# JihyongOh/DeMFI

Measured on AMD Instinct MI355X. Metric: interpolated frames/sec @720p x8 MFI (N_tst=3), higher is better.
Workload: dtype f16

## Files before the change

demfi_amd/csrc/conv_wstream.hip:

```cpp
#include "conv_common.h"

namespace {

#ifndef DEMFI_WS3_DEPTH
#define DEMFI_WS3_DEPTH 9
#endif
#ifndef DEMFI_WS_NW
#define DEMFI_WS_NW 4
#endif
template <int KS, int NW, int NCH = 2, int TH_ = 16> struct WsCfg {
    static constexpr int TH = TH_;
    static constexpr int RPW = TH / (NW / NCH);
    static constexpr int BL = KS + RPW - 1;
    static constexpr int LH = TH + KS - 1;
    static constexpr int LL = KS == 7 ? ((TW + KS - 1 + 7) & ~7) : TW + KS - 1;
    static constexpr int NI = (LH * LL + 15) / 16;
    static constexpr int UNIT_BYTES = NI * 1024;
    static constexpr int LDS_BYTES = 2 * UNIT_BYTES;
    static constexpr int NG = 2 * KS;
    static constexpr int NSTEP = NG * KS;
    static constexpr int DEPTH = NW == 8 ? KS : (KS == 7 ? 2 * KS : DEMFI_WS3_DEPTH);
    static constexpr int NIW = (NI + NW - 1) / NW;
    static constexpr int DMA_EVERY = KS == 7 ? 6 : 1;
    static constexpr int DMA_PER = KS == 7 ? 1 : 3;
    static constexpr bool PIECE_STRIDES = KS != 7;
    static_assert(LDS_BYTES <= 160 * 1024, "two units must fit LDS");
    static_assert((NIW + DMA_PER - 1) / DMA_PER * DMA_EVERY + DEPTH <= NSTEP, "the unit's DMA must be older than the last A fragment consumed in the unit");
    static_assert(NSTEP % DEPTH == 0, "static ring indices");
};

template <int KS, int NW, int NCH = 2, int TH_ = 16>
__global__ __launch_bounds__(64 * NW, 1) void conv_wstream_c64_kernel(const demfi_conv* __restrict__ d)
{
    using C = WsCfg<KS, NW, NCH, TH_>;
    constexpr int WS_TH = C::TH;
    constexpr int RPW = C::RPW;
    extern __shared__ __attribute__((aligned(16))) char smem[];
    const int tid = threadIdx.x;
    const int lane = tid & 63;
    const int wave = __builtin_amdgcn_readfirstlane(tid >> 6);
    const int hi = lane >> 5, lx = lane & 31;
    const int cs = NCH == 2 ? (wave & 1) : 0, rh = NCH == 2 ? (wave >> 1) : wave;
    const int H = d->H, W = d->W;
    const int tiles_x = (W + TW - 1) / TW, tiles_y = (H + WS_TH - 1) / WS_TH, tiles_img = tiles_x * tiles_y;
    const int total = tiles_img * d->batch;
    int t_first, t_end, t_step;
    {
        const int G = gridDim.x;
        if ((G & 7) == 0 && total >= G) {
            const int xcd = blockIdx.x & 7, idx = blockIdx.x >> 3;
            const int q = (total + 7) >> 3, lo = xcd * q;
            t_first = lo + idx;
            t_end = min(lo + q, total);
            t_step = G >> 3;
        } else {
            t_first = blockIdx.x;
            t_end = total;
            t_step = G;
        }
    }
    if (t_first >= t_end) return;
    const int upt = d->n_chunks;
    const int n_units = ((t_end - t_first + t_step - 1) / t_step) * upt;

    const demfi_piece& p0 = d->pieces[d->chunks[0].first_piece];
    const int64_t sxb = p0.v.sx * 2, syb = p0.v.sy * 2, sbb = p0.v.sb * 2;
    const char* const zeros = (const char*)d->zero_page;
    const uint4* const wbase = (const uint4*)d->wpack;

    int doff[C::NIW], dlc[C::NIW];
#pragma unroll
    for (int j = 0; j < C::NIW; ++j) {
        const int rec = min((wave + NW * j) * 16 + (lane >> 2), C::LH * C::LL - 1);
        const int l = rec / C::LL, c = rec - l * C::LL;
        doff[j] = C::PIECE_STRIDES ? (((lane & 3) ^ ((c >> 2) & 3)) << 4) : (int)(l * syb + c * sxb) + (((lane & 3) ^ ((c >> 2) & 3)) << 4);
        dlc[j] = l | (c << 8);
    }
    int boff[C::NG];
#pragma unroll
    for (int g = 0; g < C::NG; ++g) {
        const int col = lx + (g >> 1);
        boff[g] = (rh * RPW * C::LL + col) * 64 + ((((g & 1) * 2 + hi) ^ ((col >> 2) & 3)) << 4);
    }

    struct Unit { const char* src; const char* w; int iy0, ix0; bool interior; int sx, sy; };
    const unsigned lane16 = lane * 16;
    auto unit_info = [&](int u) {
        Unit r;
        const int k = u / upt, cu = u - k * upt;
        const int it = t_first + k * t_step;
        const int bimg = it / tiles_img, rem = it - bimg * tiles_img;
        const int ty = rem / tiles_x, tx = rem - ty * tiles_x;
        r.iy0 = ty * WS_TH - KS / 2;
        r.ix0 = tx * TW - KS / 2;
        const demfi_piece& pc = d->pieces[d->chunks[cu].first_piece];
        r.sx = C::PIECE_STRIDES ? (int)(pc.v.sx * 2) : (int)sxb;
        r.sy = C::PIECE_STRIDES ? (int)(pc.v.sy * 2) : (int)syb;
        r.src = (const char*)pc.v.ptr + bimg * (C::PIECE_STRIDES ? pc.v.sb * 2 : sbb) + (int64_t)r.iy0 * r.sy + (int64_t)r.ix0 * r.sx;
        r.w = (const char*)(wbase + d->chunks[cu].w_off + cs * 64);
        r.interior = r.iy0 >= 0 && r.iy0 + C::LH <= H && r.ix0 >= 0 && r.ix0 + C::LL <= W;
        return r;
    };
    auto dma_one = [&](auto J, const Unit& un, char* buf) {
        constexpr int j = decltype(J)::value;
        const int i = wave + NW * j;
        if (i >= C::NI) return;
        const char* g = un.src + doff[j];
        if constexpr (C::PIECE_STRIDES) g += (dlc[j] & 255) * un.sy + (dlc[j] >> 8) * un.sx;
        if (!un.interior) {
            const int iy = un.iy0 + (dlc[j] & 255), ix = un.ix0 + (dlc[j] >> 8);
            if (!(iy >= 0 && iy < H && ix >= 0 && ix < W)) g = zeros;
        }
        const unsigned la = (unsigned)(uintptr_t)(__attribute__((address_space(3))) char*)(buf + i * 1024);
#if defined(__HIP_DEVICE_COMPILE__)
        unsigned m0_save;
        asm volatile("s_mov_b32 %0, m0\n\ts_mov_b32 m0, %2\n\ts_nop 0\n\tglobal_load_lds_dwordx4 %1, off\n\ts_mov_b32 m0, %0"
                     : "=&s"(m0_save) : "v"(g), "s"(la) : "memory");
#endif
    };
    auto a_load = [&](const Unit& un, int t) {
        const int g = t / KS, ky = t - g * KS, kx = g >> 1, ksl = g & 1;
        return __builtin_bit_cast(uint4, *gcp<u4_t>(un.w + (unsigned)((((ky * KS + kx) * 2 + ksl) * NCH) * 1024 + lane16)));
    };

    const demfi_seg& sg = d->segs[d->sub_seg[0]];
    half_t* const dstp = (half_t*)sg.dst.ptr;
    const int act = sg.act;
    const int ch0 = d->oct_ch[0];
    f4_t bq[4];
#pragma unroll
    for (int qd = 0; qd < 4; ++qd) bq[qd] = *gcp<f4_t>(d->bias + cs * 32 + qd * 8 + hi * 4);

    f16x_t acc[RPW];
#pragma unroll
    for (int p = 0; p < RPW; ++p) {
#pragma unroll
        for (int i = 0; i < 16; ++i) acc[p][i] = 0.0f;
    }
    uint4 A[C::DEPTH];
    Unit cur = unit_info(0);
    static_for<0, C::NIW>([&](auto J) { dma_one(J, cur, smem); });
    static_for<0, C::DEPTH>([&](auto T) { A[decltype(T)::value] = a_load(cur, decltype(T)::value); });
    asm volatile("s_waitcnt vmcnt(%0)" ::"n"(C::DEPTH) : "memory");
    asm volatile("s_barrier" ::: "memory");

    for (int u = 0; u < n_units; ++u) {
        const bool has_next = u + 1 < n_units;
        TRACE_STAMP(wave, u / upt, u % upt);
        const Unit nxt = unit_info(has_next ? u + 1 : 0);
        const char* const tb = smem + (u & 1) * C::UNIT_BYTES;
        char* const nb = smem + ((u + 1) & 1) * C::UNIT_BYTES;
        uint4 B[2][C::BL];
#pragma unroll
        for (int r = 0; r < RPW; ++r) B[0][r] = *(const uint4*)(tb + boff[0] + r * (C::LL * 64));
        __builtin_amdgcn_sched_barrier(0);
        static_for<0, C::NSTEP>([&](auto T_) {
            constexpr int t = decltype(T_)::value;
            constexpr int g = t / KS, ky = t % KS, gb = g & 1;
            const uint4 a = A[t % C::DEPTH];
            if constexpr (ky + RPW < C::BL) B[gb][ky + RPW] = *(const uint4*)(tb + boff[g] + (ky + RPW) * (C::LL * 64));
            if constexpr (g + 1 < C::NG) {
                if constexpr (ky < RPW) B[gb ^ 1][ky] = *(const uint4*)(tb + boff[g + 1] + ky * (C::LL * 64));
                if constexpr (ky == KS - 1) {
#pragma unroll
                    for (int r = KS; r < RPW; ++r) B[gb ^ 1][r] = *(const uint4*)(tb + boff[g + 1] + r * (C::LL * 64));
                }
            }
            if constexpr (t + C::DEPTH < C::NSTEP) A[t % C::DEPTH] = a_load(cur, t + C::DEPTH);
            else                                   A[t % C::DEPTH] = a_load(nxt, t + C::DEPTH - C::NSTEP);
            if constexpr (KS == 7) {
                if constexpr (t % C::DMA_EVERY == 2 && t / C::DMA_EVERY < C::NIW) {
                    if (has_next) dma_one(std::integral_constant<int, t / C::DMA_EVERY>{}, nxt, nb);
                }
            } else {
                if (has_next) {
                    static_for<0, C::DMA_PER>([&](auto Q) {
                        constexpr int j = t * C::DMA_PER + decltype(Q)::value;
                        if constexpr (j < C::NIW) dma_one(std::integral_constant<int, j>{}, nxt, nb);
                    });
                }
            }
#pragma unroll
            for (int p = 0; p < RPW; ++p) Mma<half_t>::run(acc[p], a, B[gb][ky + p]);
            __builtin_amdgcn_sched_barrier(0);
        });
        asm volatile("s_waitcnt vmcnt(%0)" ::"n"(C::DEPTH) : "memory");
        const int k = u / upt;
        if (u - k * upt == upt - 1) {
            const int it = t_first + k * t_step;
            const int bimg = it / tiles_img, rem = it - bimg * tiles_img;
            const int ty = rem / tiles_x, tx = rem - ty * tiles_x;
            const int ox = tx * TW + lx;
#pragma unroll
            for (int p = 0; p < RPW; ++p) {
                const int oy = ty * WS_TH + rh * RPW + p;
#pragma unroll
                for (int m2 = 0; m2 < 2; ++m2) {
                    float v[8];
#pragma unroll
                    for (int j = 0; j < 4; ++j) {
                        v[j] = acc[p][(2 * m2) * 4 + j] + bq[2 * m2][j];
                        v[4 + j] = acc[p][(2 * m2 + 1) * 4 + j] + bq[2 * m2 + 1][j];
                    }
                    apply_act_n<8>(v, act);
                    if (oy < H && ox < W)
                        store8<half_t>(dstp + bimg * sg.dst.sb + oy * sg.dst.sy + ox * sg.dst.sx + ch0 + cs * 32 + m2 * 16 + hi * 8, v);
                }
#pragma unroll
                for (int i = 0; i < 16; ++i) acc[p][i] = 0.0f;
            }
        }
        asm volatile("s_barrier" ::: "memory");
        cur = nxt;
    }
}

static bool wstream_eligible(const demfi_conv* h, int ks = 7, int nch = 2)
{
    if (h->dtype != DEMFI_F16 || h->stride != 1 || h->kh != ks || h->kw != ks || h->pad_y != ks / 2 || h->pad_x != ks / 2) return false;
    if (h->inH != h->H || h->inW != h->W || !h->zero_page || h->rec_bytes != 64) return false;
    if (h->n_chunks < (ks == 7 ? 1 : 2) || h->cout_pad != 32 * nch || h->nco != nch) return false;
    const demfi_piece& p0 = h->pieces[h->chunks[0].first_piece];
    for (int c = 0; c < h->n_chunks; ++c) {
        const demfi_chunk& ch = h->chunks[c];
        if (ch.n_pieces != 1 || ch.nks != 2) return false;
        const demfi_piece& p = h->pieces[ch.first_piece];
        if (!p.fat || p.nch != 32 || p.up_shift || !p.v.ptr || p.v.sc != 1 || p.v.is_f32) return false;
        if (ks == 7 && (p.v.sx != p0.v.sx || p.v.sy != p0.v.sy || p.v.sb != p0.v.sb)) return false;
        if (p.v.sy * 2 * 40 >= (int64_t)1 << 31 || p.v.sx * 2 * 48 >= (int64_t)1 << 31) return false;
    }
    const int sgi = h->sub_seg[0];
    if (sgi < 0 || (nch == 2 && (h->sub_seg[1] != sgi || h->oct_ch[4] != h->oct_ch[0] + 32))) return false;
    for (int o = 0; o < 4 * nch; ++o)
        if (h->oct_seg[o] != sgi || h->oct_n[o] != 8 || h->oct_ch[o] != h->oct_ch[0] + 8 * o) return false;
    const demfi_seg& sg = h->segs[sgi];
    if (sg.mode != DEMFI_MODE_STORE || sg.scale != 1 || sg.dy || sg.dx || sg.res.ptr || !sg.dst.ptr || sg.dst.is_f32 || sg.dst.sc != 1) return false;
    return true;
}

static int launch_wstream3(const demfi_conv* h, const demfi_conv* dev, hipStream_t st)
{
    DEMFI_LDS_ATTR((conv_wstream_c64_kernel<3, 4, 1, 32>));
    const int total = ((h->W + TW - 1) / TW) * ((h->H + 31) / 32) * h->batch;
    const int grid = total >= 256 ? 256 : total;
    constexpr size_t lds = WsCfg<3, 4, 1, 32>::LDS_BYTES;
    hipLaunchKernelGGL((conv_wstream_c64_kernel<3, 4, 1, 32>), dim3(grid), dim3(256), lds, st, dev);
    DEMFI_HIP_CHECK(hipGetLastError());
    return DEMFI_OK;
}

static int launch_wstream(const demfi_conv* h, const demfi_conv* dev, hipStream_t st)
{
    DEMFI_LDS_ATTR((conv_wstream_c64_kernel<7, DEMFI_WS_NW>));
    const int total = ((h->W + TW - 1) / TW) * ((h->H + 15) / 16) * h->batch;
    const int grid = total >= 256 ? 256 : total;
    constexpr size_t lds = WsCfg<7, DEMFI_WS_NW>::LDS_BYTES;
    hipLaunchKernelGGL((conv_wstream_c64_kernel<7, DEMFI_WS_NW>), dim3(grid), dim3(64 * DEMFI_WS_NW), lds, st, dev);
    DEMFI_HIP_CHECK(hipGetLastError());
    return DEMFI_OK;
}


}

DEMFI_TU_TRACE(demfi_wstream_trace_collect)

bool demfi_wstream_eligible(const demfi_conv* h, int ks, int nch) { return wstream_eligible(h, ks, nch); }
int demfi_wstream_launch(const demfi_conv* h, const demfi_conv* dev, hipStream_t st) { return launch_wstream(h, dev, st); }
int demfi_wstream3_launch(const demfi_conv* h, const demfi_conv* dev, hipStream_t st) { return launch_wstream3(h, dev, st); }
```

Before: 105.0.

## Switch wstream conv to 16x16x32 MFMA with per-kx A-fragment prefetch queue

Replaces the 32x32 MFMA tiling of the 7x7/3x3 c64 streaming conv with 16x16x32 f16 MFMAs, splitting each wave's output into two 16-column halves and two 16-channel blocks. Weight (A) fragments are now loaded per kx column as a full set of 2*KS fragments, held in a lookahead queue of LA kx steps instead of the old per-step ring of DEPTH. Lane-to-channel mapping, B offsets, bias loads and the epilogue store are remapped to match, with 4-wide half stores. This aims for better MFMA/LDS scheduling and latency hiding, at the cost of more MFMA instructions, more A registers, and narrower output stores.

```diff
diff --git a/demfi_amd/csrc/conv_wstream.hip b/demfi_amd/csrc/conv_wstream.hip
--- a/demfi_amd/csrc/conv_wstream.hip
+++ b/demfi_amd/csrc/conv_wstream.hip
@@ -2,9 +2,6 @@
 
 namespace {
 
-#ifndef DEMFI_WS3_DEPTH
-#define DEMFI_WS3_DEPTH 9
-#endif
 #ifndef DEMFI_WS_NW
 #define DEMFI_WS_NW 4
 #endif
@@ -19,15 +16,21 @@
     static constexpr int LDS_BYTES = 2 * UNIT_BYTES;
     static constexpr int NG = 2 * KS;
     static constexpr int NSTEP = NG * KS;
-    static constexpr int DEPTH = NW == 8 ? KS : (KS == 7 ? 2 * KS : DEMFI_WS3_DEPTH);
+    static constexpr int NFR = 2 * KS;
+    static constexpr int LA = NW == 8 ? 1 : (KS == 7 ? 1 : 2);
     static constexpr int NIW = (NI + NW - 1) / NW;
     static constexpr int DMA_EVERY = KS == 7 ? 6 : 1;
     static constexpr int DMA_PER = KS == 7 ? 1 : 3;
     static constexpr bool PIECE_STRIDES = KS != 7;
     static_assert(LDS_BYTES <= 160 * 1024, "two units must fit LDS");
-    static_assert((NIW + DMA_PER - 1) / DMA_PER * DMA_EVERY + DEPTH <= NSTEP, "the unit's DMA must be older than the last A fragment consumed in the unit");
-    static_assert(NSTEP % DEPTH == 0, "static ring indices");
+    static_assert(((NIW + DMA_PER - 1) / DMA_PER - 1) * DMA_EVERY + (KS == 7 ? 2 : 0) + LA * NFR <= NSTEP,
+                  "the unit's DMA must be older than the next unit's A fragments loaded in this unit");
 };
+
+__device__ __forceinline__ void mma16(f4_t& acc, const uint4& a, const uint4& b)
+{
+    acc = __builtin_amdgcn_mfma_f32_16x16x32_f16(__builtin_bit_cast(h8_t, a), __builtin_bit_cast(h8_t, b), acc, 0, 0, 0);
+}
 
 template <int KS, int NW, int NCH = 2, int TH_ = 16>
 __global__ __launch_bounds__(64 * NW, 1) void conv_wstream_c64_kernel(const demfi_conv* __restrict__ d)
@@ -35,11 +38,12 @@
     using C = WsCfg<KS, NW, NCH, TH_>;
     constexpr int WS_TH = C::TH;
     constexpr int RPW = C::RPW;
+    constexpr int LA = C::LA, NFR = C::NFR;
     extern __shared__ __attribute__((aligned(16))) char smem[];
     const int tid = threadIdx.x;
     const int lane = tid & 63;
     const int wave = __builtin_amdgcn_readfirstlane(tid >> 6);
-    const int hi = lane >> 5, lx = lane & 31;
+    const int q4 = lane >> 4, l16 = lane & 15;
     const int cs = NCH == 2 ? (wave & 1) : 0, rh = NCH == 2 ? (wave >> 1) : wave;
     const int H = d->H, W = d->W;
     const int tiles_x = (W + TW - 1) / TW, tiles_y = (H + WS_TH - 1) / WS_TH, tiles_img = tiles_x * tiles_y;
@@ -79,12 +83,12 @@
     int boff[C::NG];
 #pragma unroll
     for (int g = 0; g < C::NG; ++g) {
-        const int col = lx + (g >> 1);
-        boff[g] = (rh * RPW * C::LL + col) * 64 + ((((g & 1) * 2 + hi) ^ ((col >> 2) & 3)) << 4);
+        const int col = (g & 1) * 16 + l16 + (g >> 1);
+        boff[g] = (rh * RPW * C::LL + col) * 64 + ((q4 ^ ((col >> 2) & 3)) << 4);
     }
 
     struct Unit { const char* src; const char* w; int iy0, ix0; bool interior; int sx, sy; };
-    const unsigned lane16 = lane * 16;
+    const unsigned aoff = (unsigned)((q4 >> 1) * NCH * 1024 + (l16 + 32 * (q4 & 1)) * 16);
     auto unit_info = [&](int u) {
         Unit r;
         const int k = u / upt, cu = u - k * upt;
@@ -118,30 +122,34 @@
                      : "=&s"(m0_save) : "v"(g), "s"(la) : "memory");
 #endif
     };
-    auto a_load = [&](const Unit& un, int t) {
-        const int g = t / KS, ky = t - g * KS, kx = g >> 1, ksl = g & 1;
-        return __builtin_bit_cast(uint4, *gcp<u4_t>(un.w + (unsigned)((((ky * KS + kx) * 2 + ksl) * NCH) * 1024 + lane16)));
+    auto a_load = [&](const Unit& un, int kx, int f) {
+        const int ky = f >> 1, cb = f & 1;
+        return __builtin_bit_cast(uint4, *gcp<u4_t>(un.w + (unsigned)((ky * KS + kx) * 2 * NCH * 1024 + cb * 256) + aoff));
     };
 
     const demfi_seg& sg = d->segs[d->sub_seg[0]];
     half_t* const dstp = (half_t*)sg.dst.ptr;
     const int act = sg.act;
     const int ch0 = d->oct_ch[0];
-    f4_t bq[4];
-#pragma unroll
-    for (int qd = 0; qd < 4; ++qd) bq[qd] = *gcp<f4_t>(d->bias + cs * 32 + qd * 8 + hi * 4);
-
-    f16x_t acc[RPW];
-#pragma unroll
-    for (int p = 0; p < RPW; ++p) {
-#pragma unroll
-        for (int i = 0; i < 16; ++i) acc[p][i] = 0.0f;
-    }
-    uint4 A[C::DEPTH];
+    f4_t bq[2];
+#pragma unroll
+    for (int cb = 0; cb < 2; ++cb) bq[cb] = *gcp<f4_t>(d->bias + cs * 32 + cb * 16 + q4 * 4);
+
+    f4_t acc[2][2][RPW];
+#pragma unroll
+    for (int cb = 0; cb < 2; ++cb)
+#pragma unroll
+        for (int h = 0; h < 2; ++h)
+#pragma unroll
+            for (int p = 0; p < RPW; ++p) acc[cb][h][p] = f4_t{0.0f, 0.0f, 0.0f, 0.0f};
+    uint4 Ac[NFR], Aq[LA][NFR], Af[NFR];
     Unit cur = unit_info(0);
     static_for<0, C::NIW>([&](auto J) { dma_one(J, cur, smem); });
-    static_for<0, C::DEPTH>([&](auto T) { A[decltype(T)::value] = a_load(cur, decltype(T)::value); });
-    asm volatile("s_waitcnt vmcnt(%0)" ::"n"(C::DEPTH) : "memory");
+    static_for<0, LA>([&](auto X) {
+#pragma unroll
+        for (int f = 0; f < NFR; ++f) Aq[decltype(X)::value][f] = a_load(cur, decltype(X)::value, f);
+    });
+    asm volatile("s_waitcnt vmcnt(%0)" ::"n"(LA * NFR) : "memory");
     asm volatile("s_barrier" ::: "memory");
 
     for (int u = 0; u < n_units; ++u) {
@@ -156,8 +164,16 @@
         __builtin_amdgcn_sched_barrier(0);
         static_for<0, C::NSTEP>([&](auto T_) {
             constexpr int t = decltype(T_)::value;
-            constexpr int g = t / KS, ky = t % KS, gb = g & 1;
-            const uint4 a = A[t % C::DEPTH];
+            constexpr int g = t / KS, ky = t % KS, gb = g & 1, kx = g >> 1, half = g & 1;
+            constexpr int f = half * KS + ky;
+            if constexpr (half == 0 && ky == 0) {
+#pragma unroll
+                for (int i = 0; i < NFR; ++i) {
+                    Ac[i] = Aq[0][i];
+#pragma unroll
+                    for (int x = 0; x + 1 < LA; ++x) Aq[x][i] = Aq[x + 1][i];
+                }
+            }
             if constexpr (ky + RPW < C::BL) B[gb][ky + RPW] = *(const uint4*)(tb + boff[g] + (ky + RPW) * (C::LL * 64));
             if constexpr (g + 1 < C::NG) {
                 if constexpr (ky < RPW) B[gb ^ 1][ky] = *(const uint4*)(tb + boff[g + 1] + ky * (C::LL * 64));
@@ -166,8 +182,6 @@
                     for (int r = KS; r < RPW; ++r) B[gb ^ 1][r] = *(const uint4*)(tb + boff[g + 1] + r * (C::LL * 64));
                 }
             }
-            if constexpr (t + C::DEPTH < C::NSTEP) A[t % C::DEPTH] = a_load(cur, t + C::DEPTH);
-            else                                   A[t % C::DEPTH] = a_load(nxt, t + C::DEPTH - C::NSTEP);
             if constexpr (KS == 7) {
                 if constexpr (t % C::DMA_EVERY == 2 && t / C::DMA_EVERY < C::NIW) {
                     if (has_next) dma_one(std::integral_constant<int, t / C::DMA_EVERY>{}, nxt, nb);
@@ -180,34 +194,47 @@
                     });
                 }
             }
-#pragma unroll
-            for (int p = 0; p < RPW; ++p) Mma<half_t>::run(acc[p], a, B[gb][ky + p]);
+            if constexpr (kx + LA < KS) Af[f] = a_load(cur, kx + LA, f);
+            else                        Af[f] = a_load(nxt, kx + LA - KS, f);
+#pragma unroll
+            for (int p = 0; p < RPW; ++p) {
+                mma16(acc[0][half][p], Ac[2 * ky], B[gb][ky + p]);
+                mma16(acc[1][half][p], Ac[2 * ky + 1], B[gb][ky + p]);
+            }
+            if constexpr (half == 1 && ky == KS - 1) {
+#pragma unroll
+                for (int i = 0; i < NFR; ++i) Aq[LA - 1][i] = Af[i];
+            }
             __builtin_amdgcn_sched_barrier(0);
         });
-        asm volatile("s_waitcnt vmcnt(%0)" ::"n"(C::DEPTH) : "memory");
+        asm volatile("s_waitcnt vmcnt(%0)" ::"n"(LA * NFR) : "memory");
         const int k = u / upt;
         if (u - k * upt == upt - 1) {
             const int it = t_first + k * t_step;
             const int bimg = it / tiles_img, rem = it - bimg * tiles_img;
             const int ty = rem / tiles_x, tx = rem - ty * tiles_x;
-            const int ox = tx * TW + lx;
+            const int cq = ch0 + cs * 32 + 8 * (q4 & 1) + 4 * (q4 >> 1);
 #pragma unroll
             for (int p = 0; p < RPW; ++p) {
                 const int oy = ty * WS_TH + rh * RPW + p;
 #pragma unroll
-                for (int m2 = 0; m2 < 2; ++m2) {
-                    float v[8];
-#pragma unroll
-                    for (int j = 0; j < 4; ++j) {
-                        v[j] = acc[p][(2 * m2) * 4 + j] + bq[2 * m2][j];
-                        v[4 + j] = acc[p][(2 * m2 + 1) * 4 + j] + bq[2 * m2 + 1][j];
+                for (int h = 0; h < 2; ++h) {
+                    const int ox = tx * TW + h * 16 + l16;
+#pragma unroll
+                    for (int cb = 0; cb < 2; ++cb) {
+                        float v[4];
+#pragma unroll
+                        for (int i = 0; i < 4; ++i) v[i] = acc[cb][h][p][i] + bq[cb][i];
+                        apply_act_n<4>(v, act);
+                        if (oy < H && ox < W) {
+                            h4_t o;
+#pragma unroll
+                            for (int i = 0; i < 4; ++i) o[i] = (half_t)v[i];
+                            *gp<h4_t>(dstp + bimg * sg.dst.sb + oy * sg.dst.sy + ox * sg.dst.sx + cq + cb * 16) = o;
+                        }
+                        acc[cb][h][p] = f4_t{0.0f, 0.0f, 0.0f, 0.0f};
                     }
-                    apply_act_n<8>(v, act);
-                    if (oy < H && ox < W)
-                        store8<half_t>(dstp + bimg * sg.dst.sb + oy * sg.dst.sy + ox * sg.dst.sx + ch0 + cs * 32 + m2 * 16 + hi * 8, v);
-                }
-#pragma unroll
-                for (int i = 0; i < 16; ++i) acc[p][i] = 0.0f;
+                }
             }
         }
         asm volatile("s_barrier" ::: "memory");
```

Result: no change. 105.4, median of 6 (+0.4%).
